# CRIMAC-WP4-Machine-learning/CRIMAC-classifiers-unet

Hardware: AMD Instinct MI355X
Metric: echogram patches/sec (4ch 256x256), training step (fwd+weighted CE+bwd+SGD) (higher is better)
Workload: dtype bf16; 1 GPU; BASELINE configs[1]: U-Net (depth 5, 64 filters) train step, batch 32 x 4x256x256 per GPU; global_batch=32, precision=bf16, start_filts=64, parallelism=dp1, ranks=1, launcher=single process

## Files before the change

crimac_classifiers_unet_amd/csrc/bnb_sums.h:

```cpp
#pragma once
#include "common.h"

namespace {

__device__ __forceinline__ void pix_split(long p, long HW, long& b, long& hw) {
  if (((p | HW) >> 31) == 0) {
    const unsigned q = (unsigned)p / (unsigned)HW;
    b = q;
    hw = (unsigned)p - q * (unsigned)HW;
  } else {
    b = p / HW;
    hw = p % HW;
  }
}

struct BnbArgs {
  const void* y;
  long y_ld;
  const float* vec;
  long stride;
  double* sum_dz;
  double* sum_dzx;
  int replicas;
};
struct BnbConst { float sc[8], sh[8], mu[8], is[8]; };
__device__ __forceinline__ void bnb_load(const BnbArgs& a, int c0, BnbConst& k) {
#pragma unroll
  for (int j = 0; j < 8; ++j) {
    k.mu[j] = a.vec[c0 + j];
    k.is[j] = a.vec[a.stride + c0 + j];
    k.sc[j] = a.vec[2 * a.stride + c0 + j];
    k.sh[j] = a.vec[3 * a.stride + c0 + j];
  }
}
template <typename T>
__device__ __forceinline__ void bnb_accum(const BnbArgs& a, const BnbConst& k, long pix, int c0, const float (&g)[8],
                                          float (&d1)[8], float (&d2)[8]) {
  float yv[8];
  load8(reinterpret_cast<const T*>(a.y) + pix * a.y_ld + c0, yv);
#pragma unroll
  for (int j = 0; j < 8; ++j) {
    const float dz = (yv[j] * k.sc[j] + k.sh[j]) > 0.f ? g[j] : 0.f;
    d1[j] += dz;
    d2[j] += dz * (yv[j] - k.mu[j]) * k.is[j];
  }
}
__device__ __forceinline__ void bnb_accum_v(const BnbConst& k, const float (&yv)[8], const float (&g)[8],
                                            float (&d1)[8], float (&d2)[8]) {
#pragma unroll
  for (int j = 0; j < 8; ++j) {
    const float dz = (yv[j] * k.sc[j] + k.sh[j]) > 0.f ? g[j] : 0.f;
    d1[j] += dz;
    d2[j] += dz * (yv[j] - k.mu[j]) * k.is[j];
  }
}
__device__ __forceinline__ void bnb_flush(const BnbArgs& a, float* lds, int C, int c0, const float (&d1)[8],
                                          const float (&d2)[8], int nthreads) {
#pragma unroll
  for (int j = 0; j < 8; ++j) {
    atomicAdd(&lds[c0 + j], d1[j]);
    atomicAdd(&lds[C + c0 + j], d2[j]);
  }
  __syncthreads();
  const long rep = (long)(blockIdx.x % (unsigned)a.replicas) * C;
  for (int c = threadIdx.x; c < C; c += nthreads) {
    atomicAdd(&a.sum_dz[rep + c], (double)lds[c]);
    atomicAdd(&a.sum_dzx[rep + c], (double)lds[C + c]);
  }
}

inline bool bnb_args_ok(const void* y, long y_ld, const float* vec, long stride, double* s0, double* s1, int replicas,
                        int C) {
  if (!s0) return true;
  return y && vec && s1 && y_ld >= C && y_ld % 8 == 0 && stride >= C && replicas >= 1;
}

}
```

crimac_classifiers_unet_amd/csrc/elementwise.hip:

```cpp
#include <stdarg.h>
#include <stdlib.h>

#include <mutex>

#include "common.h"
#include "bnb_sums.h"

static thread_local char g_err[512] = "";
void crimac_set_error(const char* fmt, ...) {
  va_list ap;
  va_start(ap, fmt);
  vsnprintf(g_err, sizeof(g_err), fmt, ap);
  va_end(ap);
}
extern "C" const char* crimac_last_error(void) { return g_err; }
extern "C" int crimac_version(void) { return CRIMAC_ABI_VERSION; }
extern "C" int crimac_layer_desc_size(void) { return (int)sizeof(crimac_layer_desc); }

namespace {

#ifdef CRIMAC_STREAM_FORWARD
#define CRIMAC_ROW(x, M) (x)
#else
#define CRIMAC_ROW(x, M) ((M) - 1 - (x))
// ... 231 lines not shown
  double s1 = 0.0, s2 = 0.0;
  if (c < C)
    for (int r = rl; r < nrep; r += 16) { s1 += sum[(long)r * C + c]; s2 += sumsq[(long)r * C + c]; }
  red[0][cl][rl] = s1;
  red[1][cl][rl] = s2;
  __syncthreads();
  if (rl != 0 || c >= C) return;
  s1 = 0.0; s2 = 0.0;
  for (int r = 0; r < 16; ++r) { s1 += red[0][cl][r]; s2 += red[1][cl][r]; }
  const double mean = s1 / (double)M;
  double var = s2 / (double)M - mean * mean;
  if (var < 0) var = 0;
  const float invstd = (float)(1.0 / sqrt(var + (double)eps));
  const float sc = gamma[c] * invstd;
  mean_o[c] = (float)mean;
  invstd_o[c] = invstd;
  scale_o[c] = sc;
  shift_o[c] = beta[c] - (float)mean * sc;
  if (rmean) {
    const double unb = M > 1 ? var * ((double)M / (double)(M - 1)) : var;
    rmean[c] = (1.f - momentum) * rmean[c] + momentum * (float)mean;
    rvar[c] = (1.f - momentum) * rvar[c] + momentum * (float)unb;
  }
}

__global__ __launch_bounds__(256) void sum_replicas_kernel(const double* __restrict__ src, int nrep,
                                                           long stride, int n, double* dst64, float* dst32,
                                                           const double* __restrict__ src_b, double* dst_b) {
  __shared__ double red[16][17];
  if (blockIdx.y == 1) { src = src_b; dst64 = dst_b; dst32 = nullptr; }
  const int cl = threadIdx.x & 15, rl = threadIdx.x >> 4;
  const int i = blockIdx.x * 16 + cl;
  double s = 0.0;
  if (i < n)
    for (int r = rl; r < nrep; r += 16) s += src[(long)r * stride + i];
  red[cl][rl] = s;
  __syncthreads();
  if (rl != 0 || i >= n) return;
  s = 0.0;
  for (int r = 0; r < 16; ++r) s += red[cl][r];
  if (dst64) dst64[i] = s;
  if (dst32) dst32[i] = (float)s;
}

struct BnFin {
  const double* sum; const double* sumsq;
  int nrep;
  long count;
  const float* gamma; const float* beta;
  float eps, momentum;
  float* rmean; float* rvar; long long* nbt;
  float* vec; long stride;
};
template <typename F>
__device__ __forceinline__ void replica_sums_block(const double* __restrict__ a, const double* __restrict__ b, int nrep,
                                                   int C, double* red, F&& fn) {
  const int tid = threadIdx.x;
  const int k = C >= 256 ? 1 : 256 / C;
  for (int cb = 0; cb < C; cb += 256) {
    const int c = cb + (k == 1 ? tid : tid % C), j = k == 1 ? 0 : tid / C;
    double s1 = 0.0, s2 = 0.0;
    if (c < C && j < k) {
      constexpr int NB = 8;
      int r = j;
      for (; r + (NB - 1) * k < nrep; r += NB * k) {
        double v1[NB], v2[NB];
#pragma unroll
        for (int u = 0; u < NB; ++u) { v1[u] = a[(long)(r + u * k) * C + c]; v2[u] = b[(long)(r + u * k) * C + c]; }
#pragma unroll
        for (int u = 0; u < NB; ++u) { s1 += v1[u]; s2 += v2[u]; }
      }
      double w1[NB], w2[NB];
#pragma unroll
      for (int u = 0; u < NB; ++u) {
        const bool in = r + u * k < nrep;
        w1[u] = in ? a[(long)(r + u * k) * C + c] : 0.0;
        w2[u] = in ? b[(long)(r + u * k) * C + c] : 0.0;
      }
#pragma unroll
      for (int u = 0; u < NB; ++u) { s1 += w1[u]; s2 += w2[u]; }
    }
    if (k > 1) {
      red[tid] = s1;
      red[256 + tid] = s2;
      __syncthreads();
      if (j == 0 && c < C) {
        s1 = 0.0; s2 = 0.0;
        for (int q = 0; q < k; ++q) { s1 += red[q * C + c]; s2 += red[256 + q * C + c]; }
      }
    }
    if (j == 0 && c < C) fn(c, s1, s2);
  }
}
__device__ __forceinline__ void bn_fin_block(const BnFin& a, int C, float* cst, double* red) {
  if (blockIdx.x == 0 && threadIdx.x == 0 && a.nbt) *a.nbt += 1;
  const bool writer = blockIdx.x == 0;
  replica_sums_block(a.sum, a.sumsq, a.nrep, C, red, [&](int c, double s1, double s2) {
    const double mean = s1 / (double)a.count;
    double var = s2 / (double)a.count - mean * mean;
    if (var < 0) var = 0;
    const float invstd = (float)(1.0 / sqrt(var + (double)a.eps));
    const float sc = a.gamma[c] * invstd;
    const float sh = a.beta[c] - (float)mean * sc;
    cst[c] = (float)mean; cst[C + c] = invstd; cst[2 * C + c] = sc; cst[3 * C + c] = sh;
    if (writer) {
      a.vec[c] = (float)mean; a.vec[a.stride + c] = invstd; a.vec[2 * a.stride + c] = sc; a.vec[3 * a.stride + c] = sh;
      if (a.rmean) {
        const double unb = a.count > 1 ? var * ((double)a.count / (double)(a.count - 1)) : var;
        a.rmean[c] = (1.f - a.momentum) * a.rmean[c] + a.momentum * (float)mean;
        a.rvar[c] = (1.f - a.momentum) * a.rvar[c] + a.momentum * (float)unb;
      }
    }
  });
  __syncthreads();
}

template <typename T, typename TO = T, bool FIN = false>
__global__ __launch_bounds__(256) void bn_act_kernel(const T* __restrict__ y, long y_ld,
                                                     const float* __restrict__ scale,
                                                     const float* __restrict__ shift, int relu,
                                                     TO* __restrict__ out, long out_ld, long M, int C, BnFin fin) {
  extern __shared__ __attribute__((aligned(16))) unsigned char bn_smem[];
  float* cst = reinterpret_cast<float*>(bn_smem + 512 * sizeof(double));
  if constexpr (FIN) bn_fin_block(fin, C, cst, reinterpret_cast<double*>(bn_smem));
  const int cpr = C / 8;
  const int rpi = 256 / cpr > 0 ? 256 / cpr : 1;
  const int chunk = threadIdx.x % cpr, rl = threadIdx.x / cpr;
  if (rl >= rpi) return;
  const int c0 = chunk * 8;
  float sc[8], sh[8];
#pragma unroll
  for (int j = 0; j < 8; ++j) {
    if constexpr (FIN) {
      sc[j] = cst[2 * C + c0 + j];
      sh[j] = cst[3 * C + c0 + j];
    } else {
      sc[j] = scale ? scale[c0 + j] : 1.f;
      sh[j] = scale ? shift[c0 + j] : 0.f;
    }
  }
  const long stride = (long)gridDim.x * rpi;
  constexpr int U = 4;
  for (long m = (long)blockIdx.x * rpi + rl; m < M; m += U * stride) {
    float v[U][8];
#pragma unroll
    for (int u = 0; u < U; ++u)
// ... 136 lines not shown
#pragma unroll
        for (int d = 0; d < 4; ++d) {
          float o[8], yv[8];
          if (ds) load8s(ds + pixq[d] * ds_ld + c0, o);
          load8(reinterpret_cast<const T*>(&yraw[d]), yv);
#pragma unroll
          for (int j = 0; j < 8; ++j) o[j] = storage_round<T>((ds ? o[j] : 0.f) + (arg[j] == d ? g[j] : 0.f));
          if (da) store8(da + pixq[d] * da_ld + c0, o);
          bnb_accum_v(k, yv, o, d1, d2);
        }
        continue;
      }
      float g[8], av[4][8], yv[4][8];
      load8s(dp + r * dp_ld + c0, g);
      long pix[4];
#pragma unroll
      for (int d = 0; d < 4; ++d) {
        pix[d] = (b * H + 2 * yp + (d >> 1)) * (long)W + 2 * xp + (d & 1);
        if constexpr (BNB) {
          load8s(reinterpret_cast<const T*>(bnb.y) + pix[d] * bnb.y_ld + c0, yv[d]);
#pragma unroll
          for (int j = 0; j < 8; ++j) av[d][j] = storage_round<TA>(fmaxf(yv[d][j] * k.sc[j] + k.sh[j], 0.f));
        } else {
          load8s(a + pix[d] * a_ld + c0, av[d]);
        }
      }
      int arg[8];
#pragma unroll
      for (int j = 0; j < 8; ++j) {
        int best = 0;
        float bv = av[0][j];
#pragma unroll
        for (int d = 1; d < 4; ++d)
          if (av[d][j] > bv) { bv = av[d][j]; best = d; }
        arg[j] = best;
      }
#pragma unroll
      for (int d = 0; d < 4; ++d) {
        float o[8];
        if (ds) load8s(ds + pix[d] * ds_ld + c0, o);
#pragma unroll
        for (int j = 0; j < 8; ++j) {
          o[j] = (ds ? o[j] : 0.f) + (arg[j] == d ? g[j] : 0.f);
          if constexpr (BNB) o[j] = storage_round<T>(o[j]);
        }
        if (da) store8(da + pix[d] * da_ld + c0, o);
        if constexpr (BNB) bnb_accum_v(k, yv[d], o, d1, d2);
      }
    }
  }
  if constexpr (BNB) bnb_flush(bnb, lds, C, c0, d1, d2, 256);
}

__device__ __forceinline__ float bn_bwd_dy(float yv, float g, float sc, float sh, float mu, float is, float k1, float k2) {
#pragma clang fp contract(off)
  const float act = __builtin_fmaf(yv, sc, sh);
  const float dz = act > 0.f ? g : 0.f;
  const float xh = (yv - mu) * is;
  return sc * __builtin_fmaf(-xh, k2, dz - k1);
}

template <typename T>
__global__ __launch_bounds__(256) void bn_bwd_reduce_kernel(const T* __restrict__ da, long da_ld,
                                                            const T* __restrict__ y, long y_ld,
                                                            const float* __restrict__ scale,
                                                            const float* __restrict__ shift,
                                                            const float* __restrict__ mean,
                                                            const float* __restrict__ invstd, long M,
                                                            int C, double* sum_dz, double* sum_dzx) {
  const int c0t = (threadIdx.x % (C / 8)) * 8;
  float sc[8], sh[8], mu[8], is[8];
#pragma unroll
  for (int j = 0; j < 8; ++j) {
    sc[j] = scale[c0t + j]; sh[j] = shift[c0t + j]; mu[j] = mean[c0t + j]; is[j] = invstd[c0t + j];
  }
  colreduce<T, double, 2>(M, C,
                          [&](long m, int c0, float (&q0)[8], float (&q1)[8]) {
                            float g[8], yv[8];
                            load8(da + m * da_ld + c0, g);
                            load8(y + m * y_ld + c0, yv);
#pragma unroll
                            for (int j = 0; j < 8; ++j) {
                              const float act = yv[j] * sc[j] + sh[j];
                              const float dz = act > 0.f ? g[j] : 0.f;
                              q0[j] = dz;
                              q1[j] = dz * (yv[j] - mu[j]) * is[j];
                            }
                          },
                          sum_dz, sum_dzx);
}

template <typename T, typename TD = T>
__global__ __launch_bounds__(256) void bn_bwd_apply_kernel(
    const T* __restrict__ da, long da_ld, const T* __restrict__ y, long y_ld,
    const float* __restrict__ scale, const float* __restrict__ shift, const float* __restrict__ mean,
    const float* __restrict__ invstd, const double* __restrict__ sum_dz,
    const double* __restrict__ sum_dzx, long M, long count, int C, TD* __restrict__ dy, long dy_ld, float* dgamma,
    float* dbeta, float* dbias) {
  if (blockIdx.x == 0) {
    for (int c = threadIdx.x; c < C; c += 256) {
      dgamma[c] = (float)sum_dzx[c];
      dbeta[c] = (float)sum_dz[c];
    }
  }
  const double invM = 1.0 / (double)count;
  const int c0t = (threadIdx.x % (C / 8)) * 8;
  float sc[8], sh[8], mu[8], is[8], k1[8], k2[8];
#pragma unroll
  for (int j = 0; j < 8; ++j) {
    sc[j] = scale[c0t + j]; sh[j] = shift[c0t + j]; mu[j] = mean[c0t + j]; is[j] = invstd[c0t + j];
    k1[j] = (float)(sum_dz[c0t + j] * invM);
    k2[j] = (float)(sum_dzx[c0t + j] * invM);
  }
// ... 1070 lines not shown
```

crimac_classifiers_unet_amd/csrc/wgrad.hip:

```cpp
#include "common.h"

CRIMAC_DIAG_DECLARE(crimac_diag_clock_wgrad)

namespace {

struct WgradParams {
  const void* f; long f_ld; int CF;
  const void* s; long s_ld; int CS;
  int B, Hf, Wf;
  float* dw;
  int tiles_y, tiles_x;
  long ntiles;
  int tiles_per_block;
  int nsplits;
  long partial_stride;
  int f_es = 2, s_es = 2;
};

__device__ __forceinline__ int swz_tr(int row) { return ((row >> 1) & 1) << 6; }

__device__ __forceinline__ bf16x4 lds_tr16(const unsigned char* p) {
  return __builtin_amdgcn_ds_read_tr16_b64_v4bf16((LDS_PTR(bf16x4))(p));
}


template <int OFF>
__device__ __forceinline__ bf16x4 lds_tr16_asm(unsigned addr) {
  bf16x4 v;
  asm volatile("ds_read_b64_tr_b16 %0, %1 offset:%2" : "=v"(v) : "v"(addr), "n"(OFF) : "memory");
  return v;
}
template <int N> __device__ __forceinline__ void wait_lgkm() {
  asm volatile("s_waitcnt lgkmcnt(%0)" :: "n"(N) : "memory");
}
__device__ __forceinline__ void tie(bf16x4& x) { asm volatile("" : "+v"(x)); }

__device__ __forceinline__ int swz16(int row) { return (((row >> 1) & 1) << 6) | (((row >> 2) & 1) << 5); }

template <int MODE, int TG>
struct WgTaps {
  static constexpr int TR = MODE == 0 ? 8 : 4;
  static constexpr int NRP = TR / 2;
  static constexpr int RS = MODE == 0 ? 18 : 64;
  static constexpr int T0 = MODE == 0 ? (TG == 0 ? 0 : 5) : (TG == 0 ? 0 : 2);
  static constexpr int N = MODE == 0 ? (TG == 0 ? 5 : 4) : 2;
  static constexpr int srow(int py, int t) {
    return MODE == 0 ? (py + t / 3) * 18 + t % 3 : (2 * py + (t >> 1)) * 32 + (t & 1) * 16;
  }
};
struct WgFrags {
  bf16x4 a[4][2];
  bf16x4 b[2][2][2];
};
// ... 1391 lines not shown
}
int teams_of(int prec, int mode) {
  return (prec == CRIMAC_PREC_BF16 || prec == CRIMAC_PREC_FP16) && mode == 0 ? 2 : 1;
}

int wgrad_run(int prec, int mode, const void* f, long f_ld, int CF, const void* s, long s_ld, int CS, int B, int Hf,
              int Wf, float* dw, long partial_stride, int target_blocks, void* stream) {
  const bool mix = prec == CRIMAC_PREC_H3F_BWD;
  if (mix) {
    CRIMAC_REQUIRE(partial_stride == 0, "wgrad (H3F_BWD): the slab form is not available");
    prec = CRIMAC_PREC_FP16;
  }
  CRIMAC_REQUIRE(prec >= CRIMAC_PREC_BF16 && prec <= CRIMAC_PREC_MAX, "wgrad: bad precision %d", prec);
  CRIMAC_REQUIRE(prec != CRIMAC_PREC_F32H3, "wgrad: F32H3 is a forward-operand mode (fp16 planes have no range for "
                 "unscaled gradients); call the backward kernels with CRIMAC_PREC_F32X3, or use CRIMAC_PREC_H3P");
  CRIMAC_REQUIRE(mode == 0 || mode == 1, "wgrad: bad mode %d", mode);
  CRIMAC_REQUIRE(CF > 0 && CF % 8 == 0 && CS > 0 && CS % 8 == 0, "wgrad: channels must be multiples of 8");
  CRIMAC_REQUIRE(f_ld >= CF && s_ld >= CS && f_ld % 8 == 0 && s_ld % 8 == 0, "wgrad: bad pixel strides");
  CRIMAC_REQUIRE(B > 0 && Hf > 0 && Wf > 0 && f && s && dw, "wgrad: bad arguments");
  CRIMAC_REQUIRE(partial_stride == 0 || partial_stride >= (long)(mode == 0 ? 9 : 4) * CF * CS,
                 "wgrad: partial slab stride %ld smaller than one dW (%d taps x %d x %d)", partial_stride,
                 mode == 0 ? 9 : 4, CF, CS);
  WgradParams p;
  p.f = f; p.f_ld = f_ld; p.CF = CF; p.s = s; p.s_ld = s_ld; p.CS = CS;
  p.B = B; p.Hf = Hf; p.Wf = Wf; p.dw = dw; p.partial_stride = partial_stride;
  if (mix) {
    if (mode == 0) p.s_es = 4; else p.f_es = 4;
    const long ldmax = f_ld > s_ld ? f_ld : s_ld;
    CRIMAC_REQUIRE((20L * Wf + 64) * ldmax * 4 < (1L << 31), "wgrad (H3F_BWD): a tile's DMA offsets exceed 32 bits");
  }
  hipStream_t st = (hipStream_t)stream;
  if (prec == CRIMAC_PREC_BF16) {
    if (mode == 0 && CS <= 16)
      return launch<bf16_t, 1, 0, true, 2>(p, target_blocks, st);
    if (mode == 0) return launch<bf16_t, 1, 0, false, 2>(p, target_blocks, st);
    return launch<bf16_t, 1, 1>(p, target_blocks, st);
  }
  if (prec == CRIMAC_PREC_FP16) {
    if (mode == 0 && CS <= 16)
      return launch<half_t, 1, 0, true, 2>(p, target_blocks, st);
    if (mode == 0) return launch<half_t, 1, 0, false, 2>(p, target_blocks, st);
    return launch<half_t, 1, 1>(p, target_blocks, st);
  }
  if (prec == CRIMAC_PREC_F32X3)
    return mode == 0 ? launch<float, 2, 0>(p, target_blocks, st) : launch<float, 2, 1>(p, target_blocks, st);
  if (prec == CRIMAC_PREC_H3P) {
    if (pp_ok(prec, mode, CF, CS, f_ld, s_ld, Wf)) return launch_pp(p, target_blocks, st);
    if (up_pp_ok(prec, mode, CF, CS, f_ld, s_ld, Wf, p.partial_stride)) return launch_up_pp(p, target_blocks, st);
    return mode == 0 ? launch<hp_t, 2, 0>(p, target_blocks, st) : launch<hp_t, 2, 1>(p, target_blocks, st);
  }
  return mode == 0 ? launch<float, 3, 0>(p, target_blocks, st) : launch<float, 3, 1>(p, target_blocks, st);
}

}

static int group_check(int prec, const crimac_wgrad_group_layer* L, int n, int B) {
  CRIMAC_REQUIRE(prec == CRIMAC_PREC_BF16 || prec == CRIMAC_PREC_FP16 || prec == CRIMAC_PREC_H3P || prec == CRIMAC_PREC_H3F_BWD,
                 "wgrad_group: 16-bit storage precisions, plane pairs and H3F_BWD only (prec=%d)", prec);
  const bool hp = prec == CRIMAC_PREC_H3P;
  const bool mix = prec == CRIMAC_PREC_H3F_BWD;
  CRIMAC_REQUIRE(L && n >= 1 && n <= CRIMAC_WGRAD_GROUP_MAX_LAYERS && B > 0, "wgrad_group: 1..%d layers", CRIMAC_WGRAD_GROUP_MAX_LAYERS);
  for (int i = 0; i < n; ++i) {
    CRIMAC_REQUIRE(L[i].CF > 0 && L[i].CF % 8 == 0 && L[i].CS >= 64 && L[i].CS % 8 == 0, "wgrad_group: layer %d: CF=%d CS=%d "
                   "(CS >= 64: the first layer keeps its own launch)", i, L[i].CF, L[i].CS);
    CRIMAC_REQUIRE(L[i].f_ld >= L[i].CF && L[i].s_ld >= L[i].CS && L[i].f_ld % 8 == 0 && L[i].s_ld % 8 == 0 && L[i].Hf > 0 && L[i].Wf > 0,
                   "wgrad_group: layer %d: bad strides / sizes", i);
    CRIMAC_REQUIRE((10L * L[i].Wf + 18) * (L[i].f_ld > L[i].s_ld ? L[i].f_ld : L[i].s_ld) * ((hp || mix) ? 4 : 2) < (1L << 31),
                   "wgrad_group: layer %d: a tile's DMA offsets exceed 32 bits", i);
    CRIMAC_REQUIRE(!hp || (L[i].CF % 64 == 0 && L[i].CS % 64 == 0), "wgrad_group: layer %d: plane pairs need whole 64-channel "
                   "tiles (CF=%d CS=%d)", i, L[i].CF, L[i].CS);
  }
  return CRIMAC_OK;
}

extern "C" int crimac_wgrad_group_layer_size(void) { return (int)sizeof(crimac_wgrad_group_layer); }

extern "C" int crimac_wgrad_group_plan(int prec, crimac_wgrad_group_layer* layers, int n_layers, int B, int items_per_layer,
                                       int* items, int cap, int* counts) {
  if (int rc = group_check(prec, layers, n_layers, B)) return rc;
  CRIMAC_REQUIRE(counts, "wgrad_group_plan: counts is NULL");
  const int target = items_per_layer > 0 ? items_per_layer : 128;
  int order[CRIMAC_WGRAD_GROUP_MAX_LAYERS];
  for (int i = 0; i < n_layers; ++i) {
    crimac_wgrad_group_layer& l = layers[i];
    l.tiles_y = cdiv(l.Hf, 8);
    l.tiles_x = cdiv(l.Wf, 16);
    l.ntiles = (long)B * l.tiles_y * l.tiles_x;
    const int ch_tiles = cdiv(l.CF, 64) * cdiv(l.CS, 64);
    long splits = target / ch_tiles;
    const long pix = (long)B * l.Hf * l.Wf;
    long max_splits = pix / 4096 > 1 ? pix / 4096 : 1;
    while (max_splits * ch_tiles < target / 2 && max_splits * 2 <= pix / 1024) max_splits *= 2;
    if (splits > max_splits) splits = max_splits;
    if (splits < 1) splits = 1;
    if (splits > l.ntiles) splits = l.ntiles;
    if (splits >= 8) splits = splits / 8 * 8;
    l.tiles_per_block = cdiv(l.ntiles, splits);
    l.nsplits = cdiv(l.ntiles, l.tiles_per_block);
    CRIMAC_REQUIRE(ch_tiles < 65536 && l.nsplits < 65536, "wgrad_group_plan: layer %d does not fit the item encoding", i);
    order[i] = i;
  }
  for (int a = 1; a < n_layers; ++a)
    for (int b = a; b > 0 && layers[order[b]].tiles_per_block > layers[order[b - 1]].tiles_per_block; --b) {
      const int t = order[b]; order[b] = order[b - 1]; order[b - 1] = t;
    }
  int n[8] = {0, 0, 0, 0, 0, 0, 0, 0};
// ... 27 lines not shown
extern "C" int crimac_wgrad_group(int prec, const crimac_wgrad_group_layer* layers, int n_layers, int B, const int* items,
                                  int cap, const int* counts, unsigned int* counters, void* stream) {
  if (int rc = group_check(prec, layers, n_layers, B)) return rc;
  CRIMAC_REQUIRE(items && counts && counters && cap > 0, "wgrad_group: bad queue arguments");
  GroupParams gp;
  for (int i = 0; i < n_layers; ++i) {
    gp.layer[i] = layers[i];
    CRIMAC_REQUIRE(layers[i].f && layers[i].s && layers[i].dw, "wgrad_group: layer %d: NULL tensor", i);
    CRIMAC_REQUIRE(layers[i].tiles_per_block > 0 && layers[i].nsplits > 0 && layers[i].ntiles == (long)B * layers[i].tiles_y * layers[i].tiles_x &&
                       layers[i].tiles_y == cdiv(layers[i].Hf, 8) && layers[i].tiles_x == cdiv(layers[i].Wf, 16),
                   "wgrad_group: layer %d was not planned for this geometry (crimac_wgrad_group_plan)", i);
  }
  gp.B = B; gp.items = items; gp.cap = cap; gp.counter = counters;
  gp.f_es = 2; gp.s_es = prec == CRIMAC_PREC_H3F_BWD ? 4 : 2;
  long total = 0;
  for (int x = 0; x < 8; ++x) {
    CRIMAC_REQUIRE(counts[x] >= 0 && counts[x] <= cap, "wgrad_group: queue %d holds %d items, capacity %d", x, counts[x], cap);
    gp.count[x] = counts[x];
    total += counts[x];
  }
  if (total == 0) return CRIMAC_OK;
  constexpr size_t lds = 4 * (size_t)((8 * 16 + ((8 + 2) * 18 + 7) / 8 * 8) * 128) + 64;
  hipStream_t st = (hipStream_t)stream;
  gp.max_items = 1;
  int per_xcd = 0;
  for (int x = 0; x < 8; ++x) if (counts[x] > per_xcd) per_xcd = counts[x];
  const int ncu = 8 * per_xcd;
  if (prec == CRIMAC_PREC_H3P) {
    static unsigned long long attr_devs = 0;
    if (crimac_first_use_on_device(&attr_devs))
      (void)hipFuncSetAttribute(reinterpret_cast<const void*>(&wgrad_pp_group_kernel), hipFuncAttributeMaxDynamicSharedMemorySize, 160 * 1024);
    hipLaunchKernelGGL(wgrad_pp_group_kernel, dim3(ncu), dim3(512), 2 * (size_t)PP_BUF + 64, st, gp);
  } else if (prec == CRIMAC_PREC_BF16) {
    static unsigned long long attr_devs = 0;
    if (crimac_first_use_on_device(&attr_devs))
      (void)hipFuncSetAttribute(reinterpret_cast<const void*>(&wgrad_group_kernel<bf16_t>), hipFuncAttributeMaxDynamicSharedMemorySize, 160 * 1024);
    hipLaunchKernelGGL(wgrad_group_kernel<bf16_t>, dim3(ncu), dim3(512), lds, st, gp);
  } else {
    static unsigned long long attr_devs = 0;
    if (crimac_first_use_on_device(&attr_devs))
      (void)hipFuncSetAttribute(reinterpret_cast<const void*>(&wgrad_group_kernel<half_t>), hipFuncAttributeMaxDynamicSharedMemorySize, 160 * 1024);
    hipLaunchKernelGGL(wgrad_group_kernel<half_t>, dim3(ncu), dim3(512), lds, st, gp);
  }
  CRIMAC_LAUNCH_CHECK();
  return CRIMAC_OK;
}

extern "C" int crimac_wgrad(int prec, int mode, const void* f, long f_ld, int CF, const void* s,
                            long s_ld, int CS, int B, int Hf, int Wf, float* dw, int target_blocks,
                            void* stream) {
  return wgrad_run(prec, mode, f, f_ld, CF, s, s_ld, CS, B, Hf, Wf, dw, 0, target_blocks, stream);
}

extern "C" int crimac_wgrad_splits(int prec, int mode, int CF, int CS, int B, int Hf, int Wf, int target_blocks) {
  if (prec < CRIMAC_PREC_BF16 || prec > CRIMAC_PREC_MAX || !(mode == 0 || mode == 1) || CF <= 0 || CS <= 0 || B <= 0 ||
      Hf <= 0 || Wf <= 0)
    return CRIMAC_ERR_INVALID;
  WgradParams p;
  p.CF = CF; p.CS = CS; p.B = B; p.Hf = Hf; p.Wf = Wf;
  plan_splits(p, mode, target_blocks, pp_ok(prec, mode, CF, CS, CF, CS, Wf) ? 2 : teams_of(prec, mode));
  return p.nsplits;
}

extern "C" int crimac_wgrad_partials(int prec, int mode, const void* f, long f_ld, int CF, const void* s,
                                     long s_ld, int CS, int B, int Hf, int Wf, float* partials, long slab_stride,
                                     int target_blocks, void* stream) {
  CRIMAC_REQUIRE(slab_stride > 0, "wgrad_partials: slab_stride must be positive");
  return wgrad_run(prec, mode, f, f_ld, CF, s, s_ld, CS, B, Hf, Wf, partials, slab_stride, target_blocks, stream);
}
```

crimac_classifiers_unet_amd/engine.py:

```python
from __future__ import annotations

import contextlib
import ctypes as C
import os

import torch

from . import hip
from .hip import Act, call, ptr


def _on_device(fn):
    import functools

    @functools.wraps(fn)
    def wrapped(self, *a, **kw):
        if getattr(self, "device", None) is None:
            self.bind()
        dev = self.device
        if dev is None or dev.type != "cuda":
            return fn(self, *a, **kw)
        with torch.cuda.device(dev):
            return fn(self, *a, **kw)
    return wrapped

BN_EPS = 1e-5
BN_MOMENTUM = 0.1
CIN_PAD = 16
NARROW_WIDTHS = (8, 16, 32)
STAT_REPLICAS = 64


def _align(n, a=64):
    return (n + a - 1) // a * a


class _ConvBlock:

    def __init__(self, conv_key, bn_key, cin, cout, cin_pad=None):
        self.conv_key, self.bn_key = conv_key, bn_key
        self.cin, self.cout = cin, cout
        self.cin_pad = cin_pad or cin
        self.idx = None
        self.narrow = False


class _UpConv:

    def __init__(self, key, cin, cout, mode="transpose"):
        self.key, self.cin, self.cout, self.mode = key, cin, cout, mode
        self.up1x1 = mode == "upsample"
        self.narrow = False


class UNetEngine:
    def __init__(self, module, precision="bf16", leader=None):
        if precision not in hip.PREC_NAMES:
            raise ValueError(f"precision must be one of {list(hip.PREC_NAMES)}, got {precision!r}")
        hip.load_library()
        self.module = module
        self.leader = leader
        self._followers = []
        if leader is not None:
            leader._followers.append(self)
        self.precision = precision
        self.prec = hip.PREC_NAMES[precision]
        self.act_dtype = {"bf16": torch.bfloat16, "fp16": torch.float16}.get(precision, torch.float32)
        self.planes = hip.PREC_PLANES[self.prec]
        self.planes_arg = hip.PREC_PLANES_ARG[self.prec]
        self.is16 = self.prec in hip.PREC_16BIT
        self.is_hp = self.prec == hip.PREC_H3P
        self.lds_dma = self.is16 or self.is_hp
        self.prec_bwd = hip.PREC_BACKWARD.get(self.prec, self.prec)
        self.loss_scale = 2.0 ** 16 if precision in ("fp16", "h3p", "h3f") else 1.0
        self.dynamic_loss_scale = precision in ("fp16", "h3p", "h3f")
        self.bwd16 = precision == "h3f"
        self.fuse_unpool_apply = precision not in ("bf16", "fp16")
        if self.bwd16:
            self.prec_bwd = hip.PREC_H3F_BWD
        self._scale_state = None
        self._skipped_seen = 0
        self._good_checks = 0
        self.depth = module.depth
# ... 896 lines not shown
                    if pool is not None:
                        self._act(b2, a2, None, pool, B, h, w, train=False)
            cur = pool if pool is not None else a2
        for j in range(D - 1):
            L = D - 2 - j
            h, w, M = geo[L]
            c = self.sf * 2 ** L
            u = self.ups[j]
            b1, b2 = self.dec[j]
            cat = self._buf(f"cat{L}", (M, 2 * c))
            up = Act(cat, c, off=0, ld=2 * c)
            catA = Act(cat, 2 * c)
            hp, wp, _ = geo[L + 1]
            self._upconv_fwd(cur, u, up, B, hp, wp)
            a1 = Act(self._buf(f"d{j}.a1", (M, c)), c)
            a2 = Act(self._buf(f"d{j}.a2", (M, c)), c)
            if training:
                y1 = Act(self._buf(f"d{j}.y1", (M, c)), c)
                y2 = Act(self._buf(f"d{j}.y2", (M, c)), c)
                self._conv_bn(b1, catA, y1, a1, None, B, h, w, M, 2 * c)
                if j == D - 2 and self.fuse_head_bn and self.fuse_bn_bwd:
                    self._conv_stats(b2, a1, y2, B, h, w, c)
                    self._bn_train(b2, y2, M)
                    head_bn = b2
                    a2 = y2
                else:
                    self._conv_bn(b2, a1, y2, a2, None, B, h, w, M, c)
                saved[f"d{j}"] = (cur, catA, y1, a1, y2, a2)
            else:
                self._conv_folded(b1, catA, a1, B, h, w, 2 * c)
                self._conv_folded(b2, a1, a2, B, h, w, c)
            cur = a2
        logits = out if out is not None else torch.empty((B, self.n_classes, H, W), dtype=torch.float32,
                                                         device=self.device)
        bn_scale, bn_shift = (ptr(self._bnf(head_bn, 2)), ptr(self._bnf(head_bn, 3))) if head_bn is not None else (None, None)
        if self.lmi:
            if meta is None:
                raise ValueError("UNet_LateMetInject needs the metadata tensor")
            call("crimac_head_meta_fwd", self.prec, cur.p, cur.ld, ptr(self.P["conv_final.weight"]),
                 ptr(self.P["conv_final.bias"]), ptr(meta), self.meta_channels, *self._mlp(), ptr(logits), B, H, W,
                 self.n_classes, 1 if softmax else 0, bn_scale, bn_shift)
            saved["meta"] = meta
        else:
            call("crimac_head_fwd", self.prec, cur.p, cur.ld, self.sf, ptr(self.P["conv_final.weight"]),
                 ptr(self.P["conv_final.bias"]), ptr(logits), B, H, W, self.n_classes, 1 if softmax else 0, bn_scale, bn_shift)
        saved["head_in"] = cur if head_bn is None else None
        self.saved = saved if training else None
        if training:
            self.forward_generation += 1
        return logits

    def _block_bwd(self, tag, b, da: Act, y: Act, x_in: Act, B, h, w, M, dx_out: Act, reduce_done=False,
                   next_bn=None, bias_from_stats=None, unpool_src=None):
        dy = self._bn_bwd(tag, b, da, y, B, h, w, M, reduce_done, unpool_src)
        self._wgrad(self.prec_bwd, 0, dy.p, dy.ld, b.cout, x_in.p, x_in.ld, b.cin_pad, B, h, w, b.conv_key,
                    flops=2.0 * 9 * b.cin * b.cout * B * h * w)
        if dx_out is None:
            return False
        return self._dgrad(tag, b, dy, dx_out, B, h, w, M, next_bn, bias_from_stats) and next_bn is not None

    def _bn_bwd(self, tag, b, da: Act, y: Act, B, h, w, M, reduce_done, unpool_src):
        world = self._sync_world()
        folded = reduce_done and self.fold_bn_finalize and world == 1
        if folded:
            pass
        elif reduce_done:
            call("crimac_sum_replicas", ptr(self._stat(b, 0)), self._nrep(b.cout), b.cout, b.cout,
                 ptr(self._stat(b, 2)), None, ptr(self._stat(b, 1)), ptr(self._stat(b, 3)))
        else:
            call("crimac_bn_bwd_reduce", self.prec, da.p, da.ld, y.p, y.ld, ptr(self._bnf(b, 2)),
                 ptr(self._bnf(b, 3)), ptr(self._bnf(b, 0)), ptr(self._bnf(b, 1)), M, b.cout,
                 ptr(self._stat(b, 2)), ptr(self._stat(b, 3)))
        dy = Act(self._buf(f"{tag}.dy", (M, b.cout), torch.float16 if self.bwd16 else None), b.cout)
        prec_apply = self.prec_bwd if self.bwd16 else self.prec
        dgamma, dbeta = self.G[b.bn_key + ".weight"], self.G[b.bn_key + ".bias"]
        if world > 1:
            import torch.distributed as dist
            dgamma.copy_(self._stat(b, 3))
            dbeta.copy_(self._stat(b, 2))
            dist.all_reduce(self._stat_pair(b), group=UNetEngine._bn_group)
            scr = self._buf("g.syncbn.scratch", (2, self.cmax), torch.float32)
            dgamma, dbeta = scr[0], scr[1]
        if unpool_src is not None:
            if not folded:
                raise RuntimeError("unpool_src needs the folded BatchNorm-backward path")
            dp_, ds_ = unpool_src
            call("crimac_unpool_bn_bwd_apply_replicas", prec_apply, dp_.p, dp_.ld, ds_.p if ds_ is not None else None,
                 ds_.ld if ds_ is not None else 0, y.p, y.ld, ptr(self._bnf(b, 0)), self.cmax, ptr(self._stat(b, 0)),
                 ptr(self._stat(b, 1)), self._nrep(b.cout), M, dy.p, dy.ld, B, h, w, b.cout, ptr(dgamma), ptr(dbeta))
        elif folded:
            call("crimac_bn_bwd_apply_replicas", prec_apply, da.p, da.ld, y.p, y.ld, ptr(self._bnf(b, 0)), self.cmax,
                 ptr(self._stat(b, 0)), ptr(self._stat(b, 1)), self._nrep(b.cout), M, M, b.cout, dy.p, dy.ld,
                 ptr(dgamma), ptr(dbeta))
        else:
            call("crimac_bn_bwd_apply", prec_apply, da.p, da.ld, y.p, y.ld, ptr(self._bnf(b, 2)),
                 ptr(self._bnf(b, 3)), ptr(self._bnf(b, 0)), ptr(self._bnf(b, 1)), ptr(self._stat(b, 2)),
                 ptr(self._stat(b, 3)), M, M * world, b.cout, dy.p, dy.ld, ptr(dgamma), ptr(dbeta), None)
        return dy

    def _dgrad_concat(self, b, dy: Act, pk, dx_up: Act, dx_out: Act, B, h, w, stats, C_up, level, side):
        self._conv3x3(dy, pk, None, dx_up, B, h, w, b.cout, b.cin, relu=False, dgrad=True, stats=stats, cols=(0, C_up),
                      out_planes=True)
        with self._fork_side(side) if side is not None else contextlib.nullcontext():
            self._conv3x3(dy, pk, None, dx_out, B, h, w, b.cout, b.cin, relu=False, dgrad=True, cols=(C_up, C_up))
            if side is not None:
                self._skip_done[level] = done = torch.cuda.Event()
                done.record()

    def _dgrad(self, tag, b, dy: Act, dx_out: Act, B, h, w, M, next_bn, bias_from_stats):
        stats, C_up, level = None, 0, None
        if bias_from_stats is not None:
            C_up, level = bias_from_stats[1:]
# ... 406 lines not shown
```

include/crimac_unet_hip.h:

```cpp
#ifndef CRIMAC_UNET_HIP_H_
#define CRIMAC_UNET_HIP_H_

#ifdef __cplusplus
extern "C" {
#endif

#define CRIMAC_OK 0
#define CRIMAC_ERR_INVALID (-22)
#define CRIMAC_ERR_LAUNCH (-5)

#define CRIMAC_PREC_BF16 0
#define CRIMAC_PREC_F32X3 1
#define CRIMAC_PREC_F32X6 2
#define CRIMAC_PREC_FP16 3
#define CRIMAC_PREC_F32H3 4
#define CRIMAC_PREC_H3P 5
#define CRIMAC_PREC_MAX 5
#define CRIMAC_PREC_H3F_BWD 6
#define CRIMAC_F32H3_WSHIFT 8
#define CRIMAC_PLANES_FWD_FP16 16
#define CRIMAC_PLANES_DG_FP16 32
#define CRIMAC_PLANES_FP16 (1 | CRIMAC_PLANES_FWD_FP16 | CRIMAC_PLANES_DG_FP16)
#define CRIMAC_PLANES_F32H3 (2 | CRIMAC_PLANES_FWD_FP16 | (CRIMAC_F32H3_WSHIFT << 8))
#define CRIMAC_PLANES_INTERLEAVED 64
#define CRIMAC_PLANES_FWD_FRAG 65536
#define CRIMAC_PLANES_DG_SCALED 128
#define CRIMAC_PLANES_H3P (2 | CRIMAC_PLANES_FWD_FP16 | CRIMAC_PLANES_DG_FP16 | CRIMAC_PLANES_INTERLEAVED | \
                           CRIMAC_PLANES_DG_SCALED | (CRIMAC_F32H3_WSHIFT << 8))

#define CRIMAC_EPI_RELU 1
#define CRIMAC_EPI_OUT_PLANES 2
#define CRIMAC_EPI_CIN4 4
#define CRIMAC_EPI_STAT_RAW 8
#define CRIMAC_EPI_WFRAG 16
#define CRIMAC_EPI_WROWS 32

#define CRIMAC_ABI_VERSION 17
int crimac_version(void);
int crimac_layer_desc_size(void);
const char* crimac_last_error(void);


int crimac_igemm_conv(int prec, const void* in, long in_ld, int B, int Hi, int Wi, int Ho, int Wo,
                      int Cin, int N, int ntaps, int tw, int pad, int stride, const void* w_hi,
                      const void* w_lo, const float* bias, int bias_mod, void* out, long out_ld,
                      int relu, int out_mode, int cout_up, void* stream);

int crimac_upconv2x2_dgrad_bnb(const void* dy, long dy_ld, int B, int H, int W, int Cout, int Cin,
                               const void* w_dg_hi, void* dx, long dx_ld, const void* bnb_y, long bnb_y_ld,
                               const float* bnb_vec, long bnb_stride, double* stat_sum, double* stat_sumsq,
                               int stat_replicas, void* stream);
int crimac_upconv2x2_dgrad_bnb_prec(int prec, const void* dy, long dy_ld, int B, int H, int W, int Cout, int Cin,
                                    const void* w_dg_hi, void* dx, long dx_ld, const void* bnb_y, long bnb_y_ld,
                                    const float* bnb_vec, long bnb_stride, double* stat_sum, double* stat_sumsq,
                                    int stat_replicas, void* stream);


int crimac_conv3x3(int prec, const void* in, long in_ld, int B, int H, int W, int Cin, int N,
                   const void* w_hi, const void* w_lo, const float* bias, void* out, long out_ld,
                   int relu, int stat_mode, double* stat_sum, double* stat_sumsq, int stat_replicas,
                   const void* bnb_y, long bnb_y_ld, const float* bnb_vec, long bnb_stride, void* stream);

int crimac_conv3x3_cols(int prec, const void* in, long in_ld, int B, int H, int W, int Cin, int N,
                   const void* w_hi, const void* w_lo, const float* bias, void* out, long out_ld,
                   int relu, int stat_mode, double* stat_sum, double* stat_sumsq, int stat_replicas,
                   const void* bnb_y, long bnb_y_ld, const float* bnb_vec, long bnb_stride, int n_first, int n_count, void* stream);

int crimac_conv3x3_pool(int prec, const void* in, long in_ld, int B, int H, int W, int Cin, int N,
                        const void* w_hi, const void* w_lo, const float* bias, void* out, long out_ld, int relu,
                        void* pool_out, long pool_ld, void* stream);

int crimac_wgrad(int prec, int mode, const void* f, long f_ld, int CF, const void* s, long s_ld,
                 int CS, int B, int Hf, int Wf, float* dw, int target_blocks, void* stream);

#define CRIMAC_WGRAD_GROUP_MAX_LAYERS 16
typedef struct crimac_wgrad_group_layer {
  const void* f; long f_ld; int CF;
  const void* s; long s_ld; int CS;
  int Hf, Wf;
  float* dw;
  int tiles_y, tiles_x;
  long ntiles;
  int tiles_per_block, nsplits;
} crimac_wgrad_group_layer;
int crimac_wgrad_group_layer_size(void);
int crimac_wgrad_group_plan(int prec, crimac_wgrad_group_layer* layers, int n_layers, int B, int items_per_layer,
                            int* items, int cap, int* counts);
int crimac_wgrad_group(int prec, const crimac_wgrad_group_layer* layers, int n_layers, int B, const int* items, int cap,
                       const int* counts, unsigned int* counters, void* stream);
int crimac_wgrad_splits(int prec, int mode, int CF, int CS, int B, int Hf, int Wf, int target_blocks);
int crimac_wgrad_partials(int prec, int mode, const void* f, long f_ld, int CF, const void* s, long s_ld, int CS,
                          int B, int Hf, int Wf, float* partials, long slab_stride, int target_blocks, void* stream);

int crimac_conv1x1_up2x(int prec, const void* x, long x_ld, int B, int H, int W, int Cin, int Cout, const void* w_hi,
                        const void* w_lo, const float* bias, void* work, void* out, long out_ld, void* stream);
int crimac_up2x_adjoint(int prec, const void* dy, long dy_ld, int B, int H, int W, int C, void* dz, long dz_ld,
                        void* stream);
int crimac_conv1x1_dgrad(int prec, const void* dz, long dz_ld, int B, int H, int W, int Cout, int Cin, const void* w_dg_hi,
                         const void* w_dg_lo, void* dx, long dx_ld, void* stream);
int crimac_conv1x1_wgrad(int prec, const void* dz, long dz_ld, int Cout, const void* x, long x_ld, int Cin, long M,
                         float* dw, void* stream);



int crimac_pack_conv3x3(const float* w, int Co, int Ci, int Ci_pad, const float* scale, int planes,
                        void* fwd_hi, void* fwd_lo, void* dg_hi, void* dg_lo, void* stream);
int crimac_pack_upconv2x2(const float* w, int Ci, int Co, int planes, void* fwd_hi, void* fwd_lo,
                          void* dg_hi, void* dg_lo, void* stream);
int crimac_unpack_wgrad_conv3x3(const float* dw, int Co, int Ci, int Ci_pad, float* grad, void* stream);
int crimac_unpack_wgrad_upconv2x2(const float* dw, int Ci, int Co, float* grad, void* stream);

typedef struct crimac_layer_desc {
  const float* w;
  float* grad;
  const float* dw;
  void* fwd_hi;
  void* fwd_lo;
  void* dg_hi;
  void* dg_lo;
  int kind;
  int Co, Ci, Ci_pad;
  int dw_splits;
  long dw_stride;
} crimac_layer_desc;
#define CRIMAC_LAYER_FWD_FRAG 16
#define CRIMAC_LAYER_DG_FRAG 32
// ... 268 lines not shown
```

Measured before the change: 2988 patches/s.

## Fuse first-layer BN backward apply with weight-gradient MFMA kernel

Adds a single kernel for the first encoder conv layer. It finalizes the BN backward reduction sums into dgamma/dbeta, computes dy from da and y on the fly, stages dy and the input halo tile in LDS (double-buffered), and accumulates the 3x3 weight gradient with MFMA, atomically adding into dw. This removes the separate BN-apply kernel, the dy round trip through global memory before the wgrad read, and one launch at the largest spatial resolution. The cost is a persistent grid of one block per CU and atomics on dw. The path is gated on a specific config: rank 1, 64 filters, cin at most 4, and 16-bit precision.

Result: no change. 2987 patches/s (-0.0%).

```diff
diff --git a/crimac_classifiers_unet_amd/csrc/bnb_sums.h b/crimac_classifiers_unet_amd/csrc/bnb_sums.h
--- a/crimac_classifiers_unet_amd/csrc/bnb_sums.h
+++ b/crimac_classifiers_unet_amd/csrc/bnb_sums.h
@@ -75,4 +75,53 @@
   return y && vec && s1 && y_ld >= C && y_ld % 8 == 0 && stride >= C && replicas >= 1;
 }
 
+template <typename F>
+__device__ __forceinline__ void replica_sums_block(const double* __restrict__ a, const double* __restrict__ b, int nrep,
+                                                   int C, double* red, F&& fn) {
+  const int tid = threadIdx.x;
+  const int k = C >= 256 ? 1 : 256 / C;
+  const bool on = tid < 256;
+  for (int cb = 0; cb < C; cb += 256) {
+    const int c = cb + (k == 1 ? tid : tid % C), j = k == 1 ? 0 : tid / C;
+    double s1 = 0.0, s2 = 0.0;
+    if (on && c < C && j < k) {
+      constexpr int NB = 8;
+      int r = j;
+      for (; r + (NB - 1) * k < nrep; r += NB * k) {
+        double v1[NB], v2[NB];
+#pragma unroll
+        for (int u = 0; u < NB; ++u) { v1[u] = a[(long)(r + u * k) * C + c]; v2[u] = b[(long)(r + u * k) * C + c]; }
+#pragma unroll
+        for (int u = 0; u < NB; ++u) { s1 += v1[u]; s2 += v2[u]; }
+      }
+      double w1[NB], w2[NB];
+#pragma unroll
+      for (int u = 0; u < NB; ++u) {
+        const bool in = r + u * k < nrep;
+        w1[u] = in ? a[(long)(r + u * k) * C + c] : 0.0;
+        w2[u] = in ? b[(long)(r + u * k) * C + c] : 0.0;
+      }
+#pragma unroll
+      for (int u = 0; u < NB; ++u) { s1 += w1[u]; s2 += w2[u]; }
+    }
+    if (k > 1) {
+      if (on) { red[tid] = s1; red[256 + tid] = s2; }
+      __syncthreads();
+      if (on && j == 0 && c < C) {
+        s1 = 0.0; s2 = 0.0;
+        for (int q = 0; q < k; ++q) { s1 += red[q * C + c]; s2 += red[256 + q * C + c]; }
+      }
+    }
+    if (on && j == 0 && c < C) fn(c, s1, s2);
+  }
 }
+
+__device__ __forceinline__ float bn_bwd_dy(float yv, float g, float sc, float sh, float mu, float is, float k1, float k2) {
+#pragma clang fp contract(off)
+  const float act = __builtin_fmaf(yv, sc, sh);
+  const float dz = act > 0.f ? g : 0.f;
+  const float xh = (yv - mu) * is;
+  return sc * __builtin_fmaf(-xh, k2, dz - k1);
+}
+
+}
diff --git a/crimac_classifiers_unet_amd/csrc/elementwise.hip b/crimac_classifiers_unet_amd/csrc/elementwise.hip
--- a/crimac_classifiers_unet_amd/csrc/elementwise.hip
+++ b/crimac_classifiers_unet_amd/csrc/elementwise.hip
@@ -307,46 +307,6 @@
   float* rmean; float* rvar; long long* nbt;
   float* vec; long stride;
 };
-template <typename F>
-__device__ __forceinline__ void replica_sums_block(const double* __restrict__ a, const double* __restrict__ b, int nrep,
-                                                   int C, double* red, F&& fn) {
-  const int tid = threadIdx.x;
-  const int k = C >= 256 ? 1 : 256 / C;
-  for (int cb = 0; cb < C; cb += 256) {
-    const int c = cb + (k == 1 ? tid : tid % C), j = k == 1 ? 0 : tid / C;
-    double s1 = 0.0, s2 = 0.0;
-    if (c < C && j < k) {
-      constexpr int NB = 8;
-      int r = j;
-      for (; r + (NB - 1) * k < nrep; r += NB * k) {
-        double v1[NB], v2[NB];
-#pragma unroll
-        for (int u = 0; u < NB; ++u) { v1[u] = a[(long)(r + u * k) * C + c]; v2[u] = b[(long)(r + u * k) * C + c]; }
-#pragma unroll
-        for (int u = 0; u < NB; ++u) { s1 += v1[u]; s2 += v2[u]; }
-      }
-      double w1[NB], w2[NB];
-#pragma unroll
-      for (int u = 0; u < NB; ++u) {
-        const bool in = r + u * k < nrep;
-        w1[u] = in ? a[(long)(r + u * k) * C + c] : 0.0;
-        w2[u] = in ? b[(long)(r + u * k) * C + c] : 0.0;
-      }
-#pragma unroll
-      for (int u = 0; u < NB; ++u) { s1 += w1[u]; s2 += w2[u]; }
-    }
-    if (k > 1) {
-      red[tid] = s1;
-      red[256 + tid] = s2;
-      __syncthreads();
-      if (j == 0 && c < C) {
-        s1 = 0.0; s2 = 0.0;
-        for (int q = 0; q < k; ++q) { s1 += red[q * C + c]; s2 += red[256 + q * C + c]; }
-      }
-    }
-    if (j == 0 && c < C) fn(c, s1, s2);
-  }
-}
 __device__ __forceinline__ void bn_fin_block(const BnFin& a, int C, float* cst, double* red) {
   if (blockIdx.x == 0 && threadIdx.x == 0 && a.nbt) *a.nbt += 1;
   const bool writer = blockIdx.x == 0;
@@ -589,13 +549,6 @@
   if constexpr (BNB) bnb_flush(bnb, lds, C, c0, d1, d2, 256);
 }
 
-__device__ __forceinline__ float bn_bwd_dy(float yv, float g, float sc, float sh, float mu, float is, float k1, float k2) {
-#pragma clang fp contract(off)
-  const float act = __builtin_fmaf(yv, sc, sh);
-  const float dz = act > 0.f ? g : 0.f;
-  const float xh = (yv - mu) * is;
-  return sc * __builtin_fmaf(-xh, k2, dz - k1);
-}
 
 template <typename T>
 __global__ __launch_bounds__(256) void bn_bwd_reduce_kernel(const T* __restrict__ da, long da_ld,
diff --git a/crimac_classifiers_unet_amd/csrc/wgrad.hip b/crimac_classifiers_unet_amd/csrc/wgrad.hip
--- a/crimac_classifiers_unet_amd/csrc/wgrad.hip
+++ b/crimac_classifiers_unet_amd/csrc/wgrad.hip
@@ -1,4 +1,5 @@
 #include "common.h"
+#include "bnb_sums.h"
 
 CRIMAC_DIAG_DECLARE(crimac_diag_clock_wgrad)
 
@@ -1496,6 +1497,193 @@
   return mode == 0 ? launch<float, 3, 0>(p, target_blocks, st) : launch<float, 3, 1>(p, target_blocks, st);
 }
 
+struct FirstBwdParams {
+  const void* da; long da_ld;
+  const void* y; long y_ld;
+  const float* bn_vec; long bn_stride;
+  const double* sum_dz; const double* sum_dzx; int nrep;
+  long count;
+  const void* x; long x_ld; int C;
+  int B, H, W, tiles_y, tiles_x;
+  int ntiles;
+  float* dw; float* dgamma; float* dbeta;
+  void* dy; long dy_ld;
+};
+constexpr int FB_F_BYTES = 256 * 128, FB_S_ROWS = 18 * 18, FB_S_BYTES = FB_S_ROWS * 32;
+constexpr int FB_BUF = FB_F_BYTES + FB_S_BYTES;
+constexpr int FB_LDS = 2 * FB_BUF + 512 * (int)sizeof(double) + 2 * 64 * (int)sizeof(float);
+
+template <typename T16> __device__ __forceinline__ u16x8 fb_pack8(const float (&v)[8]) {
+  u16x8 r;
+#pragma unroll
+  for (int i = 0; i < 8; ++i) r[i] = E16<T16>::bits(v[i]);
+  return r;
+}
+
+template <typename T16>
+__global__ __launch_bounds__(512) __attribute__((amdgpu_waves_per_eu(2, 2)))
+void first_layer_bwd_kernel(FirstBwdParams p) {
+  constexpr int CF = 64;
+  extern __shared__ __attribute__((aligned(16))) unsigned char smem[];
+  double* red = reinterpret_cast<double*>(smem + 2 * FB_BUF);
+  float* k12 = reinterpret_cast<float*>(smem + 2 * FB_BUF + 512 * sizeof(double));
+  const int tid = threadIdx.x, lane = tid & 63;
+  const int wave = __builtin_amdgcn_readfirstlane(tid >> 6);
+  const T16* dap = reinterpret_cast<const T16*>(p.da);
+  const T16* yp = reinterpret_cast<const T16*>(p.y);
+  const T16* xp = reinterpret_cast<const T16*>(p.x);
+  T16* dyp = reinterpret_cast<T16*>(p.dy);
+
+  {
+    const double invM = 1.0 / (double)p.count;
+    const bool writer = blockIdx.x == 0;
+    replica_sums_block(p.sum_dz, p.sum_dzx, p.nrep, CF, red, [&](int c, double s1, double s2) {
+      k12[c] = (float)(s1 * invM);
+      k12[CF + c] = (float)(s2 * invM);
+      if (writer) { p.dbeta[c] = (float)s1; p.dgamma[c] = (float)s2; }
+    });
+    __syncthreads();
+  }
+  const int u = tid & 7, pr = tid >> 3, c0 = u * 8;
+  float sc[8], sh[8], mu[8], is[8], k1[8], k2[8];
+#pragma unroll
+  for (int j = 0; j < 8; ++j) {
+    mu[j] = p.bn_vec[c0 + j]; is[j] = p.bn_vec[p.bn_stride + c0 + j];
+    sc[j] = p.bn_vec[2 * p.bn_stride + c0 + j]; sh[j] = p.bn_vec[3 * p.bn_stride + c0 + j];
+    k1[j] = k12[c0 + j]; k2[j] = k12[CF + c0 + j];
+  }
+
+  u16x8 ga[4], gy[4];
+  u32x4 gx[2];
+  auto tile_geo = [&](int tile, int& b, int& y0, int& x0) {
+    const unsigned tt = (unsigned)tile / (unsigned)p.tiles_x;
+    x0 = (int)((unsigned)tile - tt * (unsigned)p.tiles_x) * 16;
+    b = (int)(tt / (unsigned)p.tiles_y);
+    y0 = (int)(tt - (unsigned)b * (unsigned)p.tiles_y) * 16;
+  };
+  auto fetch = [&](int b, int y0, int x0) {
+#pragma unroll
+    for (int i = 0; i < 4; ++i) {
+      const int row = pr + 64 * i, yy = y0 + (row >> 4), xx = x0 + (row & 15);
+      ga[i] = u16x8{0, 0, 0, 0, 0, 0, 0, 0};
+      gy[i] = u16x8{0, 0, 0, 0, 0, 0, 0, 0};
+      if (yy < p.H && xx < p.W) {
+        const long pix = ((long)b * p.H + yy) * p.W + xx;
+        ga[i] = __builtin_nontemporal_load(reinterpret_cast<const u16x8*>(dap + pix * p.da_ld + c0));
+        gy[i] = __builtin_nontemporal_load(reinterpret_cast<const u16x8*>(yp + pix * p.y_ld + c0));
+      }
+    }
+#pragma unroll
+    for (int i = 0; i < 2; ++i) {
+      const int e = tid + 512 * i, hrow = e >> 1, hy = hrow / 18, hx = hrow - hy * 18;
+      const int yy = y0 - 1 + hy, xx = x0 - 1 + hx;
+      gx[i] = u32x4{0, 0, 0, 0};
+      if (e < 2 * FB_S_ROWS && yy >= 0 && yy < p.H && xx >= 0 && xx < p.W)
+        gx[i] = *reinterpret_cast<const u32x4*>(xp + (((long)b * p.H + yy) * p.W + xx) * p.x_ld + (e & 1) * 8);
+    }
+  };
+  auto stage = [&](int b, int y0, int x0, int buf) {
+    unsigned char* sF = smem + buf * FB_BUF;
+    unsigned char* sS = sF + FB_F_BYTES;
+#pragma unroll
+    for (int i = 0; i < 4; ++i) {
+      const int row = pr + 64 * i, yy = y0 + (row >> 4), xx = x0 + (row & 15);
+      float g[8], yv[8], o[8];
+      load8(reinterpret_cast<const T16*>(&ga[i]), g);
+      load8(reinterpret_cast<const T16*>(&gy[i]), yv);
+#pragma unroll
+      for (int j = 0; j < 8; ++j) o[j] = bn_bwd_dy(yv[j], g[j], sc[j], sh[j], mu[j], is[j], k1[j], k2[j]);
+      u16x8 r = fb_pack8<T16>(o);
+      if (!(yy < p.H && xx < p.W)) r = u16x8{0, 0, 0, 0, 0, 0, 0, 0};
+      else if (dyp) __builtin_nontemporal_store(r, reinterpret_cast<u16x8*>(dyp + (((long)b * p.H + yy) * p.W + xx) * p.dy_ld + c0));
+      *(LDS_PTR(u16x8))(sF + row * 128 + ((u * 16) ^ swz16(row))) = r;
+    }
+#pragma unroll
+    for (int i = 0; i < 2; ++i) {
+      const int e = tid + 512 * i;
+      if (e < 2 * FB_S_ROWS) *(LDS_PTR(u32x4))(sS + e * 16) = gx[i];
+    }
+  };
+
+  const int g = lane >> 4, li = lane & 15, q = li >> 2, pp = li & 3;
+  const int fh = wave & 3, kh = wave >> 2;
+  const int RF = (g >> 1) * 16 + 4 * (g & 1) + q;
+  const int RS = (g >> 1) * 18 + 4 * (g & 1) + q;
+  const int f_off = (RF * 128 + 8 * pp + swz16(RF)) ^ (fh << 5);
+  const int s_off = RS * 32 + 8 * pp;
+  f32x4 acc[9];
+  acc_zero(acc);
+
+  const int stride = (int)gridDim.x;
+  int tile = (int)blockIdx.x, b = 0, y0 = 0, x0 = 0;
+  if (tile < p.ntiles) {
+    tile_geo(tile, b, y0, x0);
+    fetch(b, y0, x0);
+  }
+  for (int it = 0; tile < p.ntiles; tile += stride, ++it) {
+    const int buf = it & 1;
+    stage(b, y0, x0, buf);
+    if (tile + stride < p.ntiles) {
+      tile_geo(tile + stride, b, y0, x0);
+      fetch(b, y0, x0);
+    }
+    group_barrier_lds();
+    const unsigned char* sF = smem + buf * FB_BUF + f_off;
+    const unsigned char* sS = smem + buf * FB_BUF + FB_F_BYTES + s_off;
+#pragma unroll
+    for (int r4 = 0; r4 < 4; ++r4) {
+      const int rp = kh * 4 + r4;
+      const bf16x4 a0 = lds_tr16(sF + rp * 32 * 128), a1 = lds_tr16(sF + (rp * 32 + 8) * 128);
+      const bf16x8 af = __builtin_shufflevector(a0, a1, 0, 1, 2, 3, 4, 5, 6, 7);
+#pragma unroll
+      for (int t = 0; t < 9; ++t) {
+        const int c = (2 * rp + t / 3) * 18 + t % 3;
+        const bf16x4 b0 = lds_tr16(sS + c * 32), b1 = lds_tr16(sS + (c + 8) * 32);
+        const bf16x8 bfr = __builtin_shufflevector(b0, b1, 0, 1, 2, 3, 4, 5, 6, 7);
+        acc[t] = E16<T16>::mfma16(af, bfr, acc[t]);
+      }
+    }
+  }
+
+  __syncthreads();
+  f32x4* xa = reinterpret_cast<f32x4*>(smem) + (fh * 9) * 64 + lane;
+  if (kh == 1) {
+#pragma unroll
+    for (int t = 0; t < 9; ++t) xa[t * 64] = acc[t];
+  }
+  __syncthreads();
+  if (kh == 1) return;
+  const int col = lane & 15;
+  if (col >= p.C) return;
+#pragma unroll
+  for (int t = 0; t < 9; ++t) {
+    const f32x4 o = xa[t * 64];
+#pragma unroll
+    for (int r = 0; r < 4; ++r) {
+      const int row = fh * 16 + (lane >> 4) * 4 + r;
+      atomicAdd(p.dw + ((long)t * CF + row) * 16 + col, acc[t][r] + o[r]);
+    }
+  }
+}
+
+template <typename T16>
+int launch_first_bwd(FirstBwdParams p, hipStream_t st) {
+  p.tiles_y = cdiv(p.H, 16);
+  p.tiles_x = cdiv(p.W, 16);
+  const long ntiles = (long)p.B * p.tiles_y * p.tiles_x;
+  CRIMAC_REQUIRE(ntiles < (1L << 30), "first_layer_bwd: %ld tiles exceed the kernel's 32-bit tile index", ntiles);
+  p.ntiles = (int)ntiles;
+  static unsigned long long attr_devs = 0;
+  if (crimac_first_use_on_device(&attr_devs))
+    (void)hipFuncSetAttribute(reinterpret_cast<const void*>(&first_layer_bwd_kernel<T16>), hipFuncAttributeMaxDynamicSharedMemorySize,
+                              160 * 1024);
+  const long ncu = crimac_cu_count();
+  const long grid = ntiles < ncu ? ntiles : ncu;
+  hipLaunchKernelGGL(first_layer_bwd_kernel<T16>, dim3((unsigned)grid), dim3(512), (size_t)FB_LDS, st, p);
+  CRIMAC_LAUNCH_CHECK();
+  return CRIMAC_OK;
+}
+
 }
 
 static int group_check(int prec, const crimac_wgrad_group_layer* L, int n, int B) {
@@ -1629,6 +1817,28 @@
   return wgrad_run(prec, mode, f, f_ld, CF, s, s_ld, CS, B, Hf, Wf, dw, 0, target_blocks, stream);
 }
 
+extern "C" int crimac_first_layer_bwd(int prec, const void* da, long da_ld, const void* y, long y_ld, const float* bn_vec,
+                                      long bn_stride, const double* sum_dz, const double* sum_dz_xhat, int replicas,
+                                      long count, const void* x, long x_ld, int C, int B, int H, int W, float* dw,
+                                      float* dgamma, float* dbeta, void* dy, long dy_ld, void* stream) {
+  CRIMAC_REQUIRE(prec == CRIMAC_PREC_BF16 || prec == CRIMAC_PREC_FP16, "first_layer_bwd: 16-bit storage only (prec=%d)", prec);
+  CRIMAC_REQUIRE(da && y && bn_vec && bn_stride >= 64 && sum_dz && sum_dz_xhat && replicas >= 1 && x && dw && dgamma && dbeta,
+                 "first_layer_bwd: bad arguments");
+  CRIMAC_REQUIRE(B > 0 && H > 0 && W > 0 && C >= 1 && C <= 16, "first_layer_bwd: bad sizes (B=%d H=%d W=%d C=%d)", B, H, W, C);
+  CRIMAC_REQUIRE(da_ld >= 64 && y_ld >= 64 && x_ld >= 16 && da_ld % 8 == 0 && y_ld % 8 == 0 && x_ld % 8 == 0,
+                 "first_layer_bwd: bad pixel strides");
+  CRIMAC_REQUIRE(!dy || (dy_ld >= 64 && dy_ld % 8 == 0), "first_layer_bwd: bad dy stride %ld", dy_ld);
+  const long M = (long)B * H * W;
+  CRIMAC_REQUIRE(count == 0 || count >= M, "first_layer_bwd: count smaller than the pixels of this call");
+  FirstBwdParams p;
+  p.da = da; p.da_ld = da_ld; p.y = y; p.y_ld = y_ld; p.bn_vec = bn_vec; p.bn_stride = bn_stride;
+  p.sum_dz = sum_dz; p.sum_dzx = sum_dz_xhat; p.nrep = replicas; p.count = count == 0 ? M : count;
+  p.x = x; p.x_ld = x_ld; p.C = C; p.B = B; p.H = H; p.W = W; p.dw = dw; p.dgamma = dgamma; p.dbeta = dbeta;
+  p.dy = dy; p.dy_ld = dy_ld;
+  if (prec == CRIMAC_PREC_BF16) return launch_first_bwd<bf16_t>(p, (hipStream_t)stream);
+  return launch_first_bwd<half_t>(p, (hipStream_t)stream);
+}
+
 extern "C" int crimac_wgrad_splits(int prec, int mode, int CF, int CS, int B, int Hf, int Wf, int target_blocks) {
   if (prec < CRIMAC_PREC_BF16 || prec > CRIMAC_PREC_MAX || !(mode == 0 || mode == 1) || CF <= 0 || CS <= 0 || B <= 0 ||
       Hf <= 0 || Wf <= 0)
diff --git a/crimac_classifiers_unet_amd/engine.py b/crimac_classifiers_unet_amd/engine.py
--- a/crimac_classifiers_unet_amd/engine.py
+++ b/crimac_classifiers_unet_amd/engine.py
@@ -29,6 +29,7 @@
 CIN_PAD = 16
 NARROW_WIDTHS = (8, 16, 32)
 STAT_REPLICAS = 64
+FUSE_FIRST_LAYER_BWD = True
 
 
 def _align(n, a=64):
@@ -1031,12 +1032,25 @@
 
     def _block_bwd(self, tag, b, da: Act, y: Act, x_in: Act, B, h, w, M, dx_out: Act, reduce_done=False,
                    next_bn=None, bias_from_stats=None, unpool_src=None):
+        if dx_out is None and unpool_src is None and self._first_layer_fused(b, reduce_done):
+            dwt = self._dw(b.conv_key)[0]
+            dy = Act(self._buf(f"{tag}.dy", (M, b.cout)), b.cout)
+            call("crimac_first_layer_bwd", self.prec_bwd, da.p, da.ld, y.p, y.ld, ptr(self._bnf(b, 0)), self.cmax,
+                 ptr(self._stat(b, 0)), ptr(self._stat(b, 1)), self._nrep(b.cout), M, x_in.p, x_in.ld, b.cin, B, h, w,
+                 ptr(dwt), ptr(self.G[b.bn_key + ".weight"]), ptr(self.G[b.bn_key + ".bias"]), dy.p, dy.ld,
+                 flops=2.0 * 9 * b.cin * b.cout * B * h * w, mfmas=hip.MFMAS_PER_PRODUCT[self.prec_bwd])
+            return False
         dy = self._bn_bwd(tag, b, da, y, B, h, w, M, reduce_done, unpool_src)
         self._wgrad(self.prec_bwd, 0, dy.p, dy.ld, b.cout, x_in.p, x_in.ld, b.cin_pad, B, h, w, b.conv_key,
                     flops=2.0 * 9 * b.cin * b.cout * B * h * w)
         if dx_out is None:
             return False
         return self._dgrad(tag, b, dy, dx_out, B, h, w, M, next_bn, bias_from_stats) and next_bn is not None
+
+    def _first_layer_fused(self, b, reduce_done):
+        return (FUSE_FIRST_LAYER_BWD and b is self.enc[0][0] and self.is16 and self.prec_bwd == self.prec
+                and reduce_done and self.fold_bn_finalize and self._sync_world() == 1 and self.sf == 64
+                and b.cin <= 4 and b.cin_pad == CIN_PAD and not b.narrow and not self.use_wgrad_partials)
 
     def _bn_bwd(self, tag, b, da: Act, y: Act, B, h, w, M, reduce_done, unpool_src):
         world = self._sync_world()
diff --git a/include/crimac_unet_hip.h b/include/crimac_unet_hip.h
--- a/include/crimac_unet_hip.h
+++ b/include/crimac_unet_hip.h
@@ -72,6 +72,11 @@
 
 int crimac_wgrad(int prec, int mode, const void* f, long f_ld, int CF, const void* s, long s_ld,
                  int CS, int B, int Hf, int Wf, float* dw, int target_blocks, void* stream);
+
+int crimac_first_layer_bwd(int prec, const void* da, long da_ld, const void* y, long y_ld, const float* bn_vec,
+                           long bn_stride, const double* sum_dz, const double* sum_dz_xhat, int replicas, long count,
+                           const void* x, long x_ld, int C, int B, int H, int W, float* dw, float* dgamma,
+                           float* dbeta, void* dy, long dy_ld, void* stream);
 
 #define CRIMAC_WGRAD_GROUP_MAX_LAYERS 16
 typedef struct crimac_wgrad_group_layer {
```
